# facebookresearch/robust_cvd

Hardware: AMD Instinct MI355X
Metric: GN/LM iterations/sec (and ms/iter) on 300-frame 384x224 video, 1/2/4/8 GPU (higher is better)
Workload: dtype f64

## Files before the change

robust_cvd_amd/csrc/cvd_host.h:

```cpp
#pragma once

#include <hip/hip_runtime.h>
#include <hip/hip_ext.h>
#include <rccl/rccl.h>
#include <rocblas/rocblas.h>
#include <rocsolver/rocsolver.h>

#include <algorithm>
#include <array>
#include <atomic>
#include <chrono>
#include <condition_variable>
#include <cmath>
#include <cstdarg>
#include <cstdint>
#include <cstdio>
#include <cstdlib>
#include <cstring>
#include <functional>
#include <limits>
#include <map>
#include <memory>
#include <mutex>
#include <set>
// ... 157 lines not shown
  DevBuf<float2> dDsrc, dDsrcOrd;
  int orderGx = -1, orderGy = -1;
  bool tableOrdered = false;
  DevBuf<unsigned char> dStatic, dInRange, dRegOwner;
  bool dense = false;
  DevBuf<float2> dFlow;
  DevBuf<unsigned char> dFMask;

  ncclComm_t comm = nullptr;
  int rank = 0, world = 1;
  std::shared_ptr<LocalGroup> localGroup;
  bool phantom = false;
  DevBuf<unsigned char> dCommStage;
  DevBuf<const unsigned char*> dCommPtrs;
  bool distForced = false;
  bool dist() const { return world > 1 || distForced; }
  int ownChunk() const { return (F + world - 1) / world; }
  int ownFirst() const { return std::min(F, rank * ownChunk()); }
  int ownCount() const { return std::min(F, (rank + 1) * ownChunk()) - ownFirst(); }
  int framesPadded() const { return dist() ? ownChunk() * world : F; }
  bool haveTriplets = false;
  std::vector<int> tripCenter;
  std::vector<long long> tripOff;
  long long tripC = 0;
  DevBuf<float> dTLoc, dTDsrc;
  DevBuf<float2> dTNdc;
  DevBuf<unsigned char> dTStatic;
  DevBuf<int> dTGroupOfC, dTCenterAll, dTCenter, dTSlot, dFtOff, dFtList;
  DevBuf<long long> dTOff;
  DevBuf<double> dCostTrip;
  std::vector<int> tripActive;
  bool tableWithTriplets = false;
  long long numValidTrip = 0;
  int qRows = 0;

  std::vector<int> itemFa, itemFb;
  std::vector<long long> itemRange;
  DevBuf<int> dItemFa, dItemFb, dItemSlot, dFiOff, dFiList, dFpOff, dFpList;
  DevBuf<AsmPart> dAsmParts;
  DevBuf<int2> dAsmUnits;
  DevBuf<double> dAsmScratch;
  DevBuf<unsigned int> dAsmCount;
  int nAsmParts = 0, nAsmSlots = 0;
  int numCU = 256;
  hipStream_t stream2 = nullptr;
  rocblas_handle rbMain = nullptr;
  DevBuf<double> dInvScratch;
  DevBuf<int> dInvInfo;
  hipEvent_t evCoarseIn = nullptr, evCoarseDone = nullptr;
  hipStream_t stream3 = nullptr;
  hipEvent_t evInvIn = nullptr, evInvDone = nullptr;
  DevBuf<FrameConst> dFc2;
  DevBuf<long long> dItemRange;
  std::vector<int> xFa, xFb;
  DevBuf<int> dXFa, dXFb, dXSlot, dXFiOff, dXPairEdge, dXDiagSlot;
  bool xDiagRows = false;
  int xRows = 0;
  DevBuf<long long> dXRange;
  DevBuf<double> dXBlocks;
  DevBuf<int> dDwPair, dDwRecOff, dXDir;
  DevBuf<double> dDwRecords, dDwGg;
  int nDwRecords = 0;
  bool denseAsList = false;
  bool denseListValid = false;
  std::vector<long long> denseListOff;
  DevBuf<int> dDlCounts;
  DevBuf<long long> dDlOffsets;
  DevBuf<unsigned int> dCounters;
  DevBuf<unsigned int> dTailBar;
  DevBuf<double> dOwnerScal;
  std::vector<unsigned char> tableRange;
  bool tableValid = false;
  bool tableIgnoresStatic = false;
  long long numValid = 0;

  std::vector<cvd_frame_pose> poses;
  cvd_xform_desc ddesc{}, sdesc{};
  std::vector<double> dparams, sparams;
  std::vector<std::array<double, 7>> poseParams;
  bool poseParamsValid = false;

  DevBuf<double> dX, dXc, dG, dLam, dMask, dScale, dDx, dR, dR1, dZ, dP0, dP1, dQ, dH, dQPart;
  DevBuf<float> dMinv;
  DevBuf<double> dFdot, dCostItem, dCostFrame, dScal, dHd, dFocal;
  DevBuf<double> dStatPart;
  DevBuf<unsigned char> dDynMask;
  DevBuf<double> dAdaptW;
  int dynW = 0, dynH = 0, adaptGx = 0, adaptGy = 0;
  bool haveDynMasks = false;
  std::shared_ptr<Frontend> frontend;

  struct CoarseHost {
    bool valid = false;
    int nEdges = 0, nBlocks = 0, nLevels = 0;
    std::vector<int> itemEdge;
    DevBuf<int> order, pos, levelPtr, levelCols, lvlBlkPtr, lvlBlks, blkCol, blkRow, colPtr, rowPtr, rowBlk, updPtr, updBlk,
        updA, updB, edgeBlk, edgeFa, edgeFb, wPtr, wRow, wtPtr, wtBlk, wtCol, wtFrame, wuPtr, wuL, wuW, itemEdgeDev, wSlot;
    DevBuf<double> edges, diag, Lb, Linv, Wb, rc, qc, y, c, dotPart, fdotY, wq, dropDiag;
    bool sparsified = false;
    bool temporalPose = false;
    int ptNn = 0, ptStepFrames = 0, ptN = 0, ptBlocks = 0;
    std::vector<int> edgeFaHost, edgeFbHost;
    DevBuf<int> ptA, ptB, ptPtr, ptList;
    DevBuf<double> ptMat, ptInv, ptR, ptT, ptDot, ptRec;
    DevBuf<TlStep> ptStepDev;
    std::vector<unsigned char> ptStepHost;
// ... 424 lines not shown
```

robust_cvd_amd/csrc/cvd_kernels.h:

```cpp
#pragma once

#include "cvd_device.h"

namespace cvd {

struct Table {
  const float4* ndc;
  const float2* dsrc;
  const int* pairA;
  const int* pairB;
  const long long* pairOff;
  const float2* flow;
  const unsigned char* fmask;
  const float* depth;
  int W, H;
  float sx, sy, invAspect;
};

__device__ __forceinline__ int densePixelOfLoc(const Table& T, float lx, float ly) {
  int px = static_cast<int>(__fmul_rn(lx, static_cast<float>(T.W)));
  int py = static_cast<int>(__fmul_rn(__fdiv_rn(ly, T.invAspect), static_cast<float>(T.H)));
  px = min(max(px, 0), T.W - 1);
  py = min(max(py, 0), T.H - 1);
  return py * T.W + px;
// ... 3 lines not shown
  if (!(isfinite(fx1) && isfinite(fy1))) return false;
  const int ix1 = static_cast<int>(__fadd_rn(fx1, 0.5f)), iy1 = static_cast<int>(__fadd_rn(fy1, 0.5f));
  if (ix1 < 0 || ix1 >= T.W || iy1 < 0 || iy1 >= T.H) return false;
  const float lx0 = __fmul_rn(static_cast<float>(ix), T.sx), ly0 = __fmul_rn(static_cast<float>(iy), T.sy);
  const float lx1 = __fmul_rn(fx1, T.sx), ly1 = __fmul_rn(fy1, T.sy);
  loc = make_float4(lx0, ly0, lx1, ly1);
  n.x = __fadd_rn(-1.f, __fmul_rn(2.f, lx0));
  n.y = __fsub_rn(1.f, __fdiv_rn(__fmul_rn(2.f, ly0), T.invAspect));
  n.z = __fadd_rn(-1.f, __fmul_rn(2.f, lx1));
  n.w = __fsub_rn(1.f, __fdiv_rn(__fmul_rn(2.f, ly1), T.invAspect));
  ai = densePixelOfLoc(T, lx0, ly0);
  bi = densePixelOfLoc(T, lx1, ly1);
  return true;
}
__device__ __forceinline__ bool denseConstraintRequest(const Table& T, int pix, int fa, int fb, float2 f, float4& n, float2& d) {
  const int iy = pix / T.W, ix = pix - iy * T.W;
  float4 loc;
  int ai, bi;
  d = make_float2(0.f, 0.f);
  if (!densePixelGeometry(T, ix, iy, f, loc, n, ai, bi)) return false;
  const size_t fs = static_cast<size_t>(T.W) * T.H;
  d.x = T.depth[fa * fs + ai];
  d.y = T.depth[fb * fs + bi];
  return true;
}
__device__ __forceinline__ bool denseDepthsValid(float2 d) { return isfinite(d.x) && d.x > 0.f && isfinite(d.y) && d.y > 0.f; }
__device__ __forceinline__ bool denseConstraintFromFlow(const Table& T, long long c, long long pixBase, int fa, int fb, float2 f,
                                                        float4& n, float2& d) {
  return denseConstraintRequest(T, static_cast<int>(c - pixBase), fa, fb, f, n, d) && denseDepthsValid(d);
}

template <bool DENSE>
__device__ __forceinline__ bool loadConstraint(const Table& T, long long c, long long pixBase, int fa, int fb, float4& n,
                                               float2& d) {
  if constexpr (!DENSE) {
    d = T.dsrc[c];
    n = T.ndc[c];
    return d.x > 0.f;
  } else {
    if (!T.fmask[c]) return false;
    return denseConstraintFromFlow(T, c, pixBase, fa, fb, T.flow[c], n, d);
  }
}

template <bool DENSE>
struct RecordStream {
  float4 ndNext;
  float2 dNext;
  __device__ __forceinline__ void prime(const Table& T, long long base, int i, int n) {
    ndNext = make_float4(0.f, 0.f, 0.f, 0.f);
    dNext = make_float2(0.f, 0.f);
    if (i < n) { dNext = (T.dsrc + base)[i]; ndNext = (T.ndc + base)[i]; }
  }
  __device__ __forceinline__ bool take(const Table& T, long long base, int i, int step, int n, long long, int, int, float4& nd,
                                       float2& d) {
    nd = ndNext;
    d = dNext;
    if (i + step < n) { dNext = (T.dsrc + base)[i + step]; ndNext = (T.ndc + base)[i + step]; }
    return d.x > 0.f;
  }
};
template <>
struct RecordStream<true> {
  float2 fNext;
  unsigned int mNext;
  __device__ __forceinline__ void prime(const Table& T, long long base, int i, int n) {
    fNext = make_float2(0.f, 0.f);
    mNext = 0u;
    if (i < n) { mNext = (T.fmask + base)[i]; fNext = (T.flow + base)[i]; }
  }
  __device__ __forceinline__ bool take(const Table& T, long long base, int i, int step, int n, long long pixBase, int fa, int fb,
                                       float4& nd, float2& d) {
    const unsigned int m = mNext;
    const float2 f = fNext;
    if (i + step < n) { mNext = (T.fmask + base)[i + step]; fNext = (T.flow + base)[i + step]; }
    if (!m) return false;
    return denseConstraintFromFlow(T, base + i, pixBase, fa, fb, f, nd, d);
  }
};

struct DenseStreamAhead {
  float2 fNext;
  unsigned int mNext;
  float4 ndCur;
  float2 dCur;
  bool candCur;
  __device__ __forceinline__ bool request(const Table& T, int pix, int fa, int fb, float2 f, float4& n, float2& d) const {
    return denseConstraintRequest(T, pix, fa, fb, f, n, d);
  }
  __device__ __forceinline__ void prime(const Table& T, long long base, int i, int step, int n, long long pixBase, int fa, int fb) {
    unsigned int m0 = 0u;
    float2 f0 = make_float2(0.f, 0.f);
    fNext = make_float2(0.f, 0.f);
    mNext = 0u;
    if (i < n) { m0 = (T.fmask + base)[i]; f0 = (T.flow + base)[i]; }
    if (i + step < n) { mNext = (T.fmask + base)[i + step]; fNext = (T.flow + base)[i + step]; }
    ndCur = make_float4(0.f, 0.f, 0.f, 0.f);
    candCur = m0 != 0u && request(T, static_cast<int>(base - pixBase) + i, fa, fb, f0, ndCur, dCur);
  }
  __device__ __forceinline__ bool take(const Table& T, long long base, int i, int step, int n, long long pixBase, int fa, int fb,
                                       float4& nd, float2& d) {
    nd = ndCur;
    d = dCur;
    const bool cand = candCur;
    const unsigned int m1 = mNext;
    const float2 f1 = fNext;
    mNext = 0u;
    if (i + 2 * step < n) { mNext = (T.fmask + base)[i + 2 * step]; fNext = (T.flow + base)[i + 2 * step]; }
    candCur = m1 != 0u && request(T, static_cast<int>(base - pixBase) + i + step, fa, fb, f1, ndCur, dCur);
    return cand && denseDepthsValid(d);
  }
};

struct Items {
  const int* fa;
  const int* fb;
  const long long* range;
  const int* slot;
  int count;
};

constexpr int kDenseFramesPerGroup = 2;
constexpr int kAsmUnit = 128;
constexpr int kAsmUnitDense = 1024;
constexpr int kDenseRun = 16;

#ifndef CVD_DETERMINISTIC
#define CVD_DETERMINISTIC 0
#endif
constexpr int kAtomicWalkers256 = CVD_DETERMINISTIC ? 64 : 256;
constexpr int kAsmThreads = CVD_DETERMINISTIC ? 64 : 512;
struct AsmPart {
  int frame;
  int u0, u1;
  int part;
  int nParts;
  int slot0;
};
struct AsmWork {
  const AsmPart* parts;
  const int2* units;
  double* scratch;
  unsigned int* counters;
};

__host__ __device__ inline int dwRecordDoubles(int G) { return 256 + 40 * G + 8; }
struct DenseRecords {
  const double* records;
  const int* recOff;
  const int* fpOff;
  const int* fpList;
};

enum : int { S_RZ = 0, S_RZOLD = 1, S_BETA = 2, S_PQ = 3, S_ALPHA = 4, S_RR = 5, S_RZ0 = 6, S_COST = 7,
             S_DG = 8, S_DR = 9, S_DLD = 10, S_DD = 11, S_XX = 12, S_NVALID = 13, S_GMAX = 14,
             S_DONE = 15, S_TARGET = 16, S_ITERS = 17,
             S_RZPART = 18,
             S_NACTIVE = 19,
             S_COUNT = 20 };

__device__ __forceinline__ double blockSumArray(const double* __restrict__ a, int n, double* red) {
  double acc = 0.0;
  for (int i = threadIdx.x; i < n; i += blockDim.x) acc += a[i];
  acc = waveSum(acc);
  __syncthreads();
  if ((threadIdx.x & 63) == 0) red[threadIdx.x >> 6] = acc;
  __syncthreads();
  double t = 0.0;
  for (int w = 0; w < (blockDim.x >> 6); ++w) t += red[w];
  __syncthreads();
  return t;
}
// ... 410 lines not shown
      dr2dDb = ((zIsMax ? 0.0 : dmx) + (zIsMin ? 0.0 : dmn)) * L.wd;
    } else {
      r2 = log(mn / mx) * L.wd;
      const double dmn = 1.0 / mn, dmx = -1.0 / mx;
      dr2dA = ((zIsMax ? dmx : 0.0) + (zIsMin ? dmn : 0.0)) * L.wd;
      dr2dDb = ((zIsMax ? 0.0 : dmx) + (zIsMin ? 0.0 : dmn)) * L.wd;
    }
  }
}

template <int SPEC>
__device__ __forceinline__ double fastRobustRho1(const Layout& L, double sq) {
  if constexpr (SPEC == 1) return rcpFast(1.0 + sq * L.cauchyC);
  else if constexpr (SPEC == 2) {
    const bool outer = sq > L.cauchyB;
    const double irt = rsqrtFast(outer ? sq : 1.0);
    return outer ? fmax(2.2250738585072014e-308, L.robustA * irt) : 1.0;
  }
  else return robustRho1(L, sq);
}
template <int SPEC>
__device__ __forceinline__ double fastRobustRho0(const Layout& L, double sq) {
  static_assert(SPEC == 1 || SPEC == 2, "the runtime choice goes through robustRho");
  if constexpr (SPEC == 1) {
    return L.cauchyB * log(1.0 + sq * L.cauchyC);
  } else {
    const bool outer = sq > L.cauchyB;
    const double irt = rsqrtFast(outer ? sq : 1.0);
    return outer ? (2.0 * L.robustA * (sq * irt) - L.cauchyB) : sq;
  }
}

__device__ __forceinline__ void fastRows(const Layout& L, double iz, double u, double vv, double ifxb, double ifyb, double& m00,
                                         double& m11, double& m02, double& m12) {
  const double wiz = L.ws * iz;
  m00 = wiz * ifxb;
  m11 = wiz * ifyb;
  m02 = wiz * u;
  m12 = wiz * vv;
}

#ifdef CVD_MV_PROFILE
__device__ unsigned long long g_mvProf[4096 * 8];
#define MV_STAMP(slot) do { if ((threadIdx.x & 63) == 0) g_mvProf[(blockIdx.x & 4095) * 8 + (slot)] = wall_clock64(); } while (0)
#else
#define MV_STAMP(slot) do {} while (0)
#endif
constexpr int kRedVals = 15;
constexpr int kRedStride = 4 * 33 + 1;

#ifndef CVD_MV_WAVES
#define CVD_MV_WAVES 4
#endif
#ifndef CVD_MV_SLOAD
#define CVD_MV_SLOAD 1
#endif
#ifndef CVD_MV_EARLY
#define CVD_MV_EARLY 1
#endif
template <int KD, int NT, int SPEC = 0, bool DENSE = false>
inline __global__ __launch_bounds__(NT) __attribute__((amdgpu_waves_per_eu(SPEC ? ((KD <= 4 && !DENSE) ? CVD_MV_WAVES : 3) : 2))) void k_matvec_pairs_fast(Layout L, Table T, Items it, const double* __restrict__ x,
                                                           const FrameConst* __restrict__ fc,
                                                           const double* __restrict__ mask,
                                                           const double* __restrict__ z, const double* __restrict__ pOld,
                                                           const double* __restrict__ scal, int useBeta,
                                                           double* __restrict__ qPart, CoarseView V) {
  const double sDone = scal[S_DONE];
  extern __shared__ __attribute__((aligned(16))) double sm[];
  constexpr int NV = KD == 1 ? kRedVals : 11;
  const int B = L.B;
  if (threadIdx.x == 0) MV_STAMP(0);
  double* xa = sm;
  double* xb = xa + B;
  double* pa = xb + B;
  double* pb = pa + B;
  double* qa = pb + B;
  double* qb = qa + B;
  FrameConst* fcs = reinterpret_cast<FrameConst*>(qb + B);
  double* red = reinterpret_cast<double*>(fcs + 2);
  double* W = red + 32;
  constexpr int kPriv = DENSE ? 8 : 1;
  constexpr bool kUsePriv = kPriv > 1;
  double* qpriv = W + static_cast<size_t>(kRedVals) * kRedStride;
  double* cl = W;
  const int item = blockIdx.x;
  const int tid = threadIdx.x;
  const int fa = it.fa[item], fb = it.fb[item];
  const double beta = useBeta ? scal[S_BETA] : 0.0;
#if CVD_MV_SLOAD
  const FrameConst* __restrict__ fcF[2] = {fc + fa, fc + fb};
#else
  const FrameConst* fcF[2] = {fcs, fcs + 1};
  {
    constexpr int FCW = sizeof(FrameConst) / 8;
    if (tid >= NT - 2 * FCW) {
      const int t = tid - (NT - 2 * FCW);
      const int which = t / FCW, k = t % FCW;
      reinterpret_cast<double*>(fcs + which)[k] = reinterpret_cast<const double*>(fc + (which ? fb : fa))[k];
    }
  }
#endif
  const long long cb0 = it.range[item * 4], ce0 = it.range[item * 4 + 1];
  constexpr bool kEarlyPrime = KD <= 4 && CVD_MV_EARLY;
  RecordStream<DENSE> rs;
  if constexpr (kEarlyPrime) rs.prime(T, cb0, (tid >> 6) * 64 + (tid & 63), static_cast<int>(ce0 - cb0));
  if (V.Wb != nullptr) {
    if (tid < 64) coarseFrameCorrection(V, fa, tid, cl);
    if (NT == 64) coarseFrameCorrection(V, fb, tid, cl + kCB);
    else if (tid >= 64 && tid < 128) coarseFrameCorrection(V, fb, tid - 64, cl + kCB);
  } else if (tid < 2 * kCB) {
    cl[tid] = (V.cF != nullptr) ? V.cF[(tid < kCB ? fa : fb) * kCB + (tid & (kCB - 1))] : 0.0;
  }
  constexpr int EPT = 256 / NT;
  double vza[EPT], vzb[EPT], vpa[EPT], vpb[EPT], vma[EPT], vmb[EPT];
  const bool tlOn = V.tl != nullptr;
  double* tls = cl + 2 * kCB;
  TlTaps tt[EPT];
  if (tlOn) {
    for (int i = tid; i < 2 * V.tlS; i += NT) {
      const int which = i >= V.tlS ? 1 : 0;
      tls[i] = V.tl[static_cast<size_t>(which ? fb : fa) * V.tlS + (i - which * V.tlS)];
    }
#pragma unroll
    for (int e = 0; e < EPT; ++e) tlLoadTaps(V, tid + e * NT, L.nD, tt[e]);
  }
#pragma unroll
  for (int e = 0; e < EPT; ++e) {
    const int i = tid + e * NT;
    vza[e] = vzb[e] = vpa[e] = vpb[e] = vma[e] = vmb[e] = 0.0;
    if (i < B) {
      const size_t ia = static_cast<size_t>(fa) * B + i, ib = static_cast<size_t>(fb) * B + i;
      xa[i] = x[ia];
      xb[i] = x[ib];
      vza[e] = z[ia];
      vzb[e] = z[ib];
      if (useBeta) { vpa[e] = pOld[ia]; vpb[e] = pOld[ib]; }
      vma[e] = mask[ia];
      vmb[e] = mask[ib];
      qa[i] = 0.0;
      qb[i] = 0.0;
    }
  }
  if constexpr (kUsePriv)
    for (int i = tid; i < kPriv * 2 * B; i += NT) qpriv[i] = 0.0;
  __syncthreads();
  if (sDone != 0.0) return;
#pragma unroll
  for (int e = 0; e < EPT; ++e) {
    const int i = tid + e * NT;
    if (i < B) {
      double ca = coarseAtLds(cl, L, i), cb2 = coarseAtLds(cl + kCB, L, i);
      if (tlOn) {
        ca += tlAt(tls, tt[e]);
        cb2 += tlAt(tls + V.tlS, tt[e]);
      }
      pa[i] = (vza[e] + ca + (useBeta ? beta * vpa[e] : 0.0)) * vma[e];
      pb[i] = (vzb[e] + cb2 + (useBeta ? beta * vpb[e] : 0.0)) * vmb[e];
    }
  }
  if (L.intrOpt == kIntrShared) {
    __syncthreads();
    if (tid == 0) {
      const double p06 = (z[6] + (useBeta ? beta * pOld[6] : 0.0)) * mask[6];
      pa[6] = p06;
      pb[6] = p06;
    }
  }
  __syncthreads();
  if (threadIdx.x == 0) MV_STAMP(1);

  const int N = SPEC ? 1 : L.N;
  const int lossType = SPEC ? static_cast<int>(kLossDisparity) : L.lossType;
  const double A = L.aspect;
  double aT[3] = {0, 0, 0}, aT0[3] = {0, 0, 0};
  double Cx[3] = {0, 0, 0};
  double aFa = 0.0, aFb = 0.0;
  double gDa[2] = {0.0, 0.0}, gDb[2] = {0.0, 0.0};
  const long long units0 = (it.range[item * 4 + 1] - it.range[item * 4] + 63) >> 6;
  for (int dir = 0; dir < 2; ++dir) {
  const long long cb = it.range[item * 4 + dir * 2], ce = it.range[item * 4 + dir * 2 + 1];
  const FrameConst& Fa = *fcF[dir];
  const FrameConst& Fb = *fcF[dir ^ 1];
  if (dir) {
    double* t;
    t = xa; xa = xb; xb = t;
    t = pa; pa = pb; pb = t;
    t = qa; qa = qb; qb = t;
#pragma unroll
    for (int i = 0; i < 3; ++i) { aT0[i] = aT[i]; aT[i] = 0.0; Cx[i] = -Cx[i]; }
    { const double o = aFa; aFa = aFb; aFb = o; }
#pragma unroll
    for (int n = 0; n < 2; ++n) { const double o = gDa[n]; gDa[n] = gDb[n]; gDb[n] = o; }
  }
  const int firstUnit = dir == 0 ? (tid >> 6) : static_cast<int>(((tid >> 6) - units0) & (NT / 64 - 1));
  const int nDir = static_cast<int>(ce - cb);
  const int iFirst = firstUnit * 64 + (tid & 63);
  if (dir || !kEarlyPrime) rs.prime(T, cb, iFirst, nDir);
  double RaU[9], RbU[9], dTU[3];
#pragma unroll
  for (int i = 0; i < 9; ++i) { RaU[i] = uniformValue(Fa.R[i]); RbU[i] = uniformValue(Fb.R[i]); }
#pragma unroll
  for (int i = 0; i < 3; ++i) dTU[i] = uniformValue(Fa.t[i] - Fb.t[i]);
  double eaU[3], ebU[3], dptU[3];
  {
    const double pwa[3] = {uniformValue(pa[3]), uniformValue(pa[4]), uniformValue(pa[5])};
    const double pwb[3] = {uniformValue(pb[3]), uniformValue(pb[4]), uniformValue(pb[5])};
#pragma unroll
    for (int k = 0; k < 3; ++k) {
      eaU[k] = uniformValue(pwa[0] * Fa.Jl[k] + pwa[1] * Fa.Jl[3 + k] + pwa[2] * Fa.Jl[6 + k]);
      ebU[k] = uniformValue(pwb[0] * Fb.Jl[k] + pwb[1] * Fb.Jl[3 + k] + pwb[2] * Fb.Jl[6 + k]);
      dptU[k] = uniformValue(pa[k] - pb[k]);
    }
  }
  const double fya = uniformValue(Fa.fy), fxa = fya * A;
  const double fyb = uniformValue(Fb.fy);
  const double ifyb = uniformValue(1.0 / fyb), ifxb = uniformValue(1.0 / (fyb * A));
  const double pfaU = uniformValue(pa[6] / fya);
  const double pfrU = uniformValue(L.ws * pb[6] * ifyb);

  const int fsrc = dir ? fb : fa, ftgt = dir ? fa : fb;
  const long long pixBase = DENSE ? (cb / (static_cast<long long>(T.W) * T.H)) * (static_cast<long long>(T.W) * T.H) : 0;
  for (int ci = iFirst; ci < nDir; ci += NT) {
    float4 nd;
    float2 d;
    if (!rs.take(T, cb, ci, NT, nDir, pixBase, fsrc, ftgt, nd, d)) continue;
    const double da = static_cast<double>(d.x), db = static_cast<double>(d.y);
    FastTaps<KD> ta, tb;
    fastGather<KD>(L, nd.x, nd.y, ta);
    fastGather<KD>(L, nd.z, nd.w, tb);
    double Da, Db, sDa, sDb;
    if (N == 0) {
      Da = da; Db = db; sDa = 0.0; sDb = 0.0;
    } else {
// ... 52 lines not shown

    const double yq0 = m00 * t0, yq1 = m11 * t1, yq2 = m02 * t0 + m12 * t1 - dr2dA * t2;
    aFb -= L.ws * (u * t0 + vv * t1);
    const double yX[3] = {RbU[0] * yq0 + RbU[1] * yq1 + RbU[2] * yq2, RbU[3] * yq0 + RbU[4] * yq1 + RbU[5] * yq2,
                          RbU[6] * yq0 + RbU[7] * yq1 + RbU[8] * yq2};
#pragma unroll
    for (int i = 0; i < 3; ++i) aT[i] += yX[i];
    Cx[0] += v[1] * yX[2] - v[2] * yX[1];
    Cx[1] += v[2] * yX[0] - v[0] * yX[2];
    Cx[2] += v[0] * yX[1] - v[1] * yX[0];
    aFa += Da * (Rcf[0] * yX[0] + Rcf[1] * yX[1] + Rcf[2] * yX[2]);
    if (N > 0) {
      const double ga = Rca[0] * yX[0] + Rca[1] * yX[1] + Rca[2] * yX[2];
      const double gb = dr2dDb * t2;
      float dxLate = d.x, dyLate = d.y;
      asm volatile("" : "+v"(dxLate), "+v"(dyLate));
      const double da = static_cast<double>(dxLate), db = static_cast<double>(dyLate);
      if constexpr (KD == 1) {
        gDa[0] += ga * da; gDa[1] += ga;
        gDb[0] += gb * db; gDb[1] += gb;
      } else {
      const int pkey = (DENSE ? tid : (tid ^ (tid >> 5))) & (kPriv - 1);
      double* qaw = kUsePriv ? qpriv + (static_cast<size_t>(pkey) * 2 + dir) * B : qa;
      double* qbw = kUsePriv ? qpriv + (static_cast<size_t>(pkey) * 2 + (dir ^ 1)) * B : qb;
      const double gad = ga * da, gbd = gb * db;
#pragma unroll
      for (int k = 0; k < KD; ++k) {
        if (ta.ok(k)) {
          const int ia = ta.I(k);
          const double wa = ta.Wt(k);
          if (N == 2) {
            atomicAdd(&qaw[7 + ia * 2], gad * wa);
            atomicAdd(&qaw[7 + ia * 2 + 1], ga * wa);
          } else {
            atomicAdd(&qaw[7 + ia], gad * wa);
          }
        }
        if (tb.ok(k)) {
          const int ib = tb.I(k);
          const double wb = tb.Wt(k);
          if (N == 2) {
            atomicAdd(&qbw[7 + ib * 2], gbd * wb);
            atomicAdd(&qbw[7 + ib * 2 + 1], gb * wb);
          } else {
            atomicAdd(&qbw[7 + ib], gbd * wb);
          }
        }
      }
      }
    }
  }
  }
  MV_STAMP(4 + ((threadIdx.x >> 6) & 3));
  const FrameConst& Fa = *fcF[1];
  const FrameConst& Fb = *fcF[0];
  {
    double vals[NV];
#pragma unroll
    for (int i = 0; i < 3; ++i) { vals[i] = aT[i]; vals[3 + i] = aT0[i]; vals[6 + i] = Cx[i]; }
    vals[9] = aFa;
    vals[10] = aFb;
    if constexpr (KD == 1) { vals[11] = gDa[0]; vals[12] = gDa[1]; vals[13] = gDb[0]; vals[14] = gDb[1]; }
    const int half = tid >> 1;
    const int colw = (half >> 5) * 33 + (half & 31);
#pragma unroll
    for (int i = 0; i < NV; ++i) {
      const double v = vals[i] + dppMove<0xB1>(vals[i]);
      if ((tid & 1) == 0) W[i * kRedStride + colw] = v;
    }
  }
  __syncthreads();
  constexpr int SEG = NT / 64;
  if (tid < NV * SEG) {
    const double* row = W + (tid / SEG) * kRedStride + (tid % SEG) * 33;
    double s0 = 0.0, s1 = 0.0, s2 = 0.0, s3 = 0.0;
#pragma unroll
    for (int k = 0; k < 32; k += 4) {
      s0 += row[k];
      s1 += row[k + 1];
      s2 += row[k + 2];
      s3 += row[k + 3];
    }
    double sacc = (s0 + s1) + (s2 + s3);
    if (SEG >= 2) sacc += dppMove<0xB1>(sacc);
    if (SEG == 4) sacc += dppMove<0x4E>(sacc);
    if (tid % SEG == 0) red[tid / SEG] = sacc;
  }
  __syncthreads();
  if (tid < 3) {
    const double d = red[tid] - red[3 + tid];
    qa[tid] += d;
    qb[tid] -= d;
  } else if (tid < 9) {
    const bool tgt = tid >= 6;
    const int i = tgt ? tid - 6 : tid - 3;
    const double dT[3] = {Fa.t[0] - Fb.t[0], Fa.t[1] - Fb.t[1], Fa.t[2] - Fb.t[2]};
    const double* y = red + (tgt ? 3 : 0);
    const double m[3] = {red[6] - (dT[1] * y[2] - dT[2] * y[1]), red[7] - (dT[2] * y[0] - dT[0] * y[2]),
                         red[8] - (dT[0] * y[1] - dT[1] * y[0])};
    const double* a = (tgt ? Fb.Jl : Fa.Jl) + 3 * i;
    const double sdot = a[0] * m[0] + a[1] * m[1] + a[2] * m[2];
    if (tgt) qb[3 + i] -= sdot;
    else qa[3 + i] += sdot;
  } else if (tid == 9) {
    qa[6] += red[9] / Fa.fy;
  } else if (tid == 10) {
    qb[6] += red[10] / Fb.fy;
  } else if (KD == 1 && tid < 15) {
    const int n = (tid - 11) & 1;
    if (n < N) {
      if (tid < 13) qa[7 + n] += red[11 + n];
      else qb[7 + n] += red[13 + n];
    }
  }
  __syncthreads();
  if (threadIdx.x == 0) MV_STAMP(2);
  { double* t = qa; qa = qb; qb = t; }
  if constexpr (kUsePriv) {
    for (int i = tid; i < B; i += NT) {
      double sa = 0.0, sb = 0.0;
#pragma unroll
      for (int k = 0; k < kPriv; ++k) {
        sa += qpriv[(static_cast<size_t>(k) * 2 + 0) * B + i];
        sb += qpriv[(static_cast<size_t>(k) * 2 + 1) * B + i];
      }
      qa[i] += sa;
      qb[i] += sb;
    }
    __syncthreads();
  }
  double* outA = qPart + static_cast<size_t>(it.slot[item * 2]) * B;
  double* outB = qPart + static_cast<size_t>(it.slot[item * 2 + 1]) * B;
  for (int i = tid; i < B; i += NT) {
    outA[i] = qa[i];
    outB[i] = qb[i];
  }
  if (threadIdx.x == 0) MV_STAMP(3);
}

}
```

robust_cvd_amd/csrc/cvd_setup.hip:

```cpp
#include "cvd_host.h"
#include "cvd_table.h"
#include "cvd_triplets.h"
#include "cvd_dense_walk.h"
#include <rocprim/device/device_segmented_radix_sort.hpp>

namespace cvd {

void launchFrameConsts(const Layout& L, const double* x, FrameConst* fc, hipStream_t s) {
  hipLaunchKernelGGL(k_frame_consts, dim3((L.F + 63) / 64), dim3(64), 0, s, L, x, fc);
}

static void quatToMatrix(const double q[4] , double R[3][3]) {
  for (int c = 0; c < 3; ++c) {
    double v[3] = {0, 0, 0};
    v[c] = 1.0;
    const double uv[3] = {2.0 * (q[1] * v[2] - q[2] * v[1]), 2.0 * (q[2] * v[0] - q[0] * v[2]),
                          2.0 * (q[0] * v[1] - q[1] * v[0])};
    R[0][c] = v[0] + q[3] * uv[0] + (q[1] * uv[2] - q[2] * uv[1]);
    R[1][c] = v[1] + q[3] * uv[1] + (q[2] * uv[0] - q[0] * uv[2]);
    R[2][c] = v[2] + q[3] * uv[2] + (q[0] * uv[1] - q[1] * uv[0]);
  }
}
static void matrixToAngleAxis(const double R[3][3], double aa[3]) {
  double q0, q1, q2, q3;
// ... 902 lines not shown
    const bool overBudget = coarseEliminationUpdates(h->F, edgeList) > updateBudget;
    {
      const int stepP = std::max(2, h->opt.coarse_temporal_step);
      const bool fits = ((h->F - 1 + stepP - 1) / stepP + 1) * kCB <= kDenseCoarseMaxUnknowns;
      const bool fusedScope = !h->dist() && h->opt.pcg_fused_tail != 0 && !h->forceGeneric && h->Bsz() <= 256 &&
                              h->opt.coarse_temporal_min_frames > 0 && h->F >= h->opt.coarse_temporal_min_frames &&
                              h->F + 2 * kTlMaxS <= 2 * h->numCU;
      h->coarse.temporalPose = fits && (h->opt.coarse_level == 3 || (overBudget && h->opt.coarse_over_budget == 0) ||
                                        (h->opt.coarse_over_budget == 0 && fusedScope));
    }
    if (h->coarse.temporalPose) {
      h->coarse.denseMode = true;
    } else if (overBudget && h->F * kCB <= denseMaxUnknowns) {
      h->coarse.denseMode = true;
    } else if (overBudget) {
      std::vector<int> newId(edgeList.size(), -1);
      std::vector<std::pair<int, int>> kept;
      for (size_t e = 0; e < edgeList.size(); ++e)
        if (coarseKeepsPair(edgeList[e].first, edgeList[e].second)) {
          newId[e] = static_cast<int>(kept.size());
          kept.push_back(edgeList[e]);
        }
      for (auto& ie : itemEdge) ie = newId[ie];
      h->coarse.sparsified = kept.size() != edgeList.size();
      edgeList.swap(kept);
    }
    buildCoarsePlan(h, edgeList, itemEdge);
    if (h->coarse.temporalPose) poseTemporalPlan(h);
    if (h->dense) {
      std::map<std::pair<int, int>, int> edgeOfPair;
      for (size_t i = 0; i < h->itemFa.size(); ++i) edgeOfPair[{h->itemFa[i], h->itemFb[i]}] = itemEdge[i];
      std::vector<int> pairEdge(std::max<size_t>(1, h->xFa.size()), -1);
      for (size_t k = 0; k < h->xFa.size(); ++k) {
        auto it = edgeOfPair.find({h->xFa[k], h->xFb[k]});
        if (it != edgeOfPair.end()) pairEdge[k] = it->second;
      }
      h->dXPairEdge.upload(pairEdge.data(), pairEdge.size(), s);
    }
  }
  std::vector<int> fiOff(h->F + 1, 0), fiList, fpOff(h->F + 1, 0), fpList;
  for (int f = 0; f < h->F; ++f) {
    fiOff[f + 1] = fiOff[f] + static_cast<int>(frameItems[f].size());
    fiList.insert(fiList.end(), frameItems[f].begin(), frameItems[f].end());
    fpOff[f + 1] = fpOff[f] + static_cast<int>(framePairs[f].size());
    fpList.insert(fpList.end(), framePairs[f].begin(), framePairs[f].end());
  }
  h->dItemFa.upload(h->itemFa.data(), h->itemFa.size(), s);
  h->dItemFb.upload(h->itemFb.data(), h->itemFb.size(), s);
  h->dItemRange.upload(h->itemRange.data(), h->itemRange.size(), s);
  std::vector<int> itemSlot(fiList.size(), 0);
  for (size_t e = 0; e < fiList.size(); ++e) itemSlot[fiList[e]] = static_cast<int>(e);
  h->qRows = static_cast<int>(fiList.size());
  h->dItemSlot.upload(itemSlot.data(), itemSlot.size(), s);
  if (withTriplets) {
    const size_t nG = h->tripActive.size();
    std::vector<long long> tOff(2 * std::max<size_t>(nG, 1), 0);
    std::vector<int> tCen(std::max<size_t>(nG, 1), 0), tSlot(3 * std::max<size_t>(nG, 1), 0);
    const int pairCodes = static_cast<int>(h->itemFa.size()) * 2;
    for (size_t k = 0; k < nG; ++k) {
      const int g = h->tripActive[k];
      tOff[2 * k] = h->tripOff[g];
      tOff[2 * k + 1] = h->tripOff[g + 1];
      tCen[k] = h->tripCenter[g];
      for (int role = 0; role < 3; ++role) tSlot[3 * k + role] = itemSlot[pairCodes + static_cast<int>(k) * 3 + role];
    }
    std::vector<int> ftOff(h->F + 1, 0), ftList;
    for (int f = 0; f < h->F; ++f) {
      ftOff[f + 1] = ftOff[f] + static_cast<int>(frameTrips[f].size());
      ftList.insert(ftList.end(), frameTrips[f].begin(), frameTrips[f].end());
    }
    h->dTOff.upload(tOff.data(), tOff.size(), s);
    h->dTCenter.upload(tCen.data(), tCen.size(), s);
    h->dTSlot.upload(tSlot.data(), tSlot.size(), s);
    h->dFtOff.upload(ftOff.data(), ftOff.size(), s);
    h->dFtList.upload(ftList.data(), ftList.size(), s);
    h->dCostTrip.ensure(std::max<size_t>(nG, 1));
  }
  {
    std::vector<int2> units;
    std::vector<int> fuOff(h->F + 1, 0);
    for (int f = 0; f < h->F; ++f) {
      for (const int code : framePairs[f]) {
        const long long n = h->pairOff[(code >> 1) + 1] - h->pairOff[code >> 1];
        for (long long o = 0; o < n; o += (h->dense ? kAsmUnitDense : kAsmUnit)) units.push_back(make_int2(code, static_cast<int>(o)));
      }
      fuOff[f + 1] = static_cast<int>(units.size());
    }
    int activeFrames = 0;
    for (int f = 0; f < h->F; ++f) activeFrames += inRange[f] ? 1 : 0;
    constexpr double partsPerCU = 1.0;
    const long long denom = std::max<long long>(1, std::max<long long>(activeFrames, static_cast<long long>(partsPerCU * h->numCU)));
    const int capU = static_cast<int>(std::max<long long>(kAsmThreads / 64, (static_cast<long long>(units.size()) + denom - 1) / denom));
    std::vector<AsmPart> parts;
    int slots = 0;
    for (int f = 0; f < h->F; ++f) {
      const int nu = fuOff[f + 1] - fuOff[f];
      const int np = std::max(1, (nu + capU - 1) / capU);
      const int per = (nu + np - 1) / np;
      for (int q = 0; q < np; ++q) {
        AsmPart a;
        a.frame = f;
        a.u0 = fuOff[f] + std::min(nu, q * per);
        a.u1 = fuOff[f] + std::min(nu, (q + 1) * per);
        a.part = q;
        a.nParts = np;
        a.slot0 = np > 1 ? slots : 0;
// ... 189 lines not shown
```

robust_cvd_amd/csrc/cvd_solve.hip:

```cpp
#include <optional>

#include "cvd_host.h"
#include "cvd_lm.h"
#include "cvd_pcg.h"
#include "cvd_coarse.h"

namespace cvd {

void launchTlRowsInit(cvd_handle* h, const TlStep* tsp, int NT, int groups, int F, unsigned int* counter, int closeScalars, double tol2,
                      hipStream_t s) {
  const size_t lds = static_cast<size_t>(tlRowsLds(NT)) * 8;
  allowLds(k_tl_rows_init, lds);
  hipLaunchKernelGGL(k_tl_rows_init, dim3(groups), dim3(768), lds, s, tsp, F, h->dScal.p, counter, closeScalars, tol2, h->hPcg);
  HIP_CHECK(hipGetLastError());
}

namespace {
struct TailStalled {};
}
static int runPcgAttempt(Ctx& c, const double* x, const std::function<void()>& tail);
int runPcg(Ctx& c, const double* x, const std::function<void()>& tail) {
  const size_t firstTimerSlot = c.h->evUsed;
  try {
    return runPcgAttempt(c, x, tail);
// ... 198 lines not shown
bool wantsTriplets(const cvd_opt_params& p, ProblemKind kind) {
  return kind == PK_POSE_STEP && (p.smooth_static_weight > 0.0 || p.smooth_dynamic_weight > 0.0);
}
void bindTriplets(Ctx& c, const cvd_opt_params& p, ProblemKind kind) {
  cvd_handle* h = c.h;
  c.trip = wantsTriplets(p, kind) && c.L.includeStatic;
  if (!c.trip) return;
  c.TT = TripletTable{h->dTNdc.p, h->dTDsrc.p, h->dTStatic.p, h->dTOff.p, h->dTCenter.p, h->dTSlot.p,
                      static_cast<int>(h->tripActive.size()),
                      static_cast<int>(p.smooth_loss_type),
                      std::sqrt(std::max(0.0, p.smooth_static_weight)), std::sqrt(std::max(0.0, p.smooth_dynamic_weight))};
}

namespace {

struct SetupPhases {
  bool on;
  double t = nowSeconds();
  void operator()(const char* what) {
    if (!on) return;
    const double now = nowSeconds();
    fprintf(stderr, "[setup] %-14s %8.1f us\n", what, (now - t) * 1e6);
    t = now;
  }
};

struct BindMode {
  bool checkBlock;
  bool staticGuards;
  bool levels;
};
struct BoundProblem {
  Ctx c;
  std::optional<DenseListScope> denseList;
};

void bindProblem(BoundProblem& b, cvd_handle* h, const cvd_opt_params& p, double depthDeformReg, ProblemKind kind,
                 const std::vector<int>& range, const BindMode& mode, SetupPhases& phase) {
  Ctx& c = b.c;
  c.h = h;
  c.L = makeLayout(h, p, depthDeformReg, kind);
  if (mode.checkBlock) checkFrameBlock(static_cast<size_t>(c.L.B), "solve");
  tapCounts(c.L, c.KD, c.KS);
  phase("layout");
  const bool guarded = !mode.staticGuards || c.L.includeStatic;
  b.denseList.emplace(h, h->dense && guarded && !denseFastScope(h, c.L, c.KS, wantsTriplets(p, kind)));
  compileTable(h, range, wantsTriplets(p, kind), kind == PK_NORMALIZE && c.L.includeStatic);
  orderTable(h, c.L, c.KD);
  phase("table");
  refreshMedians(h);
  phase("medians");
  c.T = makeTable(h);
  c.nItems = static_cast<int>(h->itemFa.size());
  c.it = Items{h->dItemFa.p, h->dItemFb.p, h->dItemRange.p, h->dItemSlot.p, c.nItems};
  c.n = static_cast<size_t>(c.L.F) * c.L.B;
  c.boundDepth0 = (kind == PK_NORMALIZE && c.L.N > 0) ? 1 : 0;
  bindTriplets(c, p, kind);
  if (guarded) checkDenseScope(h, c.L, c.KS, c.trip);
  c.cross = crossScope(h, c);
  h->coarseOn = mode.levels && h->opt.coarse_level != 0 && h->coarse.valid && c.L.includeStatic && h->coarse.nEdges > 0 &&
                !h->forceGeneric && kind == PK_POSE_STEP;
  ensureBuffers(c);
  phase("buffers");
  if (mode.levels) {
    h->coarse.ptInvPending = false;
    h->temporal.on = temporalScope(c);
    if (h->temporal.on) h->temporal.on = temporalPrepare(c);
    phase("level 3 tables");
    if (h->coarseOn && h->coarse.temporalPose) poseTemporalPrepare(c);
    phase("level 2 tables");
  }
  buildMask(h, c.L, p, kind, range);
  phase("mask");
  uploadState(h, c.L, h->dX);
  phase("upload");
}

long long countResidualBlocks(const Ctx& c, const std::vector<int>& range) {
  const cvd_handle* h = c.h;
  const long long nr = static_cast<long long>(range.size());
  long long blocks = c.trip ? h->numValidTrip : 0;
  if (c.L.scaleRegSqrt > 0.0) blocks += nr * c.L.sregX * c.L.sregY;
  if (c.L.focalRegSqrt > 0.0) blocks += nr;
  if (c.L.depthDeformW > 0.0 && c.L.depthType == CVD_DEPTH_GRID) blocks += nr;
  if (c.L.spatialDeformW > 0.0 && c.L.nS > 0) blocks += nr;
  if (c.L.positionRegSqrt > 0.0)
    for (int k = c.L.firstFrame; k < c.L.lastFrame - 1; ++k)
      blocks += (h->tableRange[k] && h->tableRange[k + 1] && h->tableRange[k + 2]) ? 1 : 0;
  return blocks;
}

struct PendingGuard {
  cvd_handle* h;
  const LevelSchedule& schedule;
  bool inverseAside = false;
  ~PendingGuard() {
    if (schedule.pending) (void)hipStreamWaitEvent(h->stream, h->evCoarseDone, 0);
    if (inverseAside) (void)hipStreamWaitEvent(h->stream, h->evInvDone, 0);
    if (h->temporal.sidePending) {
      (void)hipStreamWaitEvent(h->stream, h->temporal.evDone, 0);
      h->temporal.sidePending = false;
    }
  }
};

void rebuildTemporalLevel(Ctx& c) {
  cvd_handle* h = c.h;
// ... 296 lines not shown
```

Before: 327.1.

## Pack per-item metadata into one cache-line record and hoist matvec prologue loads

Per-item frame indices, output slots and constraint ranges now live in one 64-byte aligned record, so the matvec kernel reads them from one cache line instead of several scattered arrays. The kernel prologue now issues every global load up front into registers before writing shared memory: x/z/pOld/mask rows, coarse and temporal coefficients, tap data and the needed FrameConst fields (t, fy, Jl). Clamped addresses keep those loads branch-free. The aim is to overlap load latency at kernel start. In exchange it adds register pressure, unconditional loads of unused data, and an extra setup upload of the record array.

Result: faster. 333.1, median of 6 (+1.8%).

```diff
diff --git a/robust_cvd_amd/csrc/cvd_host.h b/robust_cvd_amd/csrc/cvd_host.h
--- a/robust_cvd_amd/csrc/cvd_host.h
+++ b/robust_cvd_amd/csrc/cvd_host.h
@@ -233,6 +233,7 @@
   hipEvent_t evInvIn = nullptr, evInvDone = nullptr;
   DevBuf<FrameConst> dFc2;
   DevBuf<long long> dItemRange;
+  DevBuf<ItemRecord> dItemRec;
   std::vector<int> xFa, xFb;
   DevBuf<int> dXFa, dXFb, dXSlot, dXFiOff, dXPairEdge, dXDiagSlot;
   bool xDiagRows = false;
diff --git a/robust_cvd_amd/csrc/cvd_kernels.h b/robust_cvd_amd/csrc/cvd_kernels.h
--- a/robust_cvd_amd/csrc/cvd_kernels.h
+++ b/robust_cvd_amd/csrc/cvd_kernels.h
@@ -79,6 +79,12 @@
     dNext = make_float2(0.f, 0.f);
     if (i < n) { dNext = (T.dsrc + base)[i]; ndNext = (T.ndc + base)[i]; }
   }
+  __device__ __forceinline__ void primeClamped(const Table& T, long long base, int i, int n) {
+    const long long c = i < n ? base + i : 0;
+    dNext = T.dsrc[c];
+    ndNext = T.ndc[c];
+    if (i >= n) { dNext = make_float2(0.f, 0.f); ndNext = make_float4(0.f, 0.f, 0.f, 0.f); }
+  }
   __device__ __forceinline__ bool take(const Table& T, long long base, int i, int step, int n, long long, int, int, float4& nd,
                                        float2& d) {
     nd = ndNext;
@@ -96,6 +102,7 @@
     mNext = 0u;
     if (i < n) { mNext = (T.fmask + base)[i]; fNext = (T.flow + base)[i]; }
   }
+  __device__ __forceinline__ void primeClamped(const Table& T, long long base, int i, int n) { prime(T, base, i, n); }
   __device__ __forceinline__ bool take(const Table& T, long long base, int i, int step, int n, long long pixBase, int fa, int fb,
                                        float4& nd, float2& d) {
     const unsigned int m = mNext;
@@ -139,12 +146,21 @@
   }
 };
 
+struct alignas(64) ItemRecord {
+  int fa, fb;
+  int slotA, slotB;
+  long long b0, e0;
+  long long b1, e1;
+  long long pad[2];
+};
+static_assert(sizeof(ItemRecord) == 64, "one record per 64-byte line");
 struct Items {
   const int* fa;
   const int* fb;
   const long long* range;
   const int* slot;
   int count;
+  const ItemRecord* rec;
 };
 
 constexpr int kDenseFramesPerGroup = 2;
@@ -661,9 +677,6 @@
 #ifndef CVD_MV_WAVES
 #define CVD_MV_WAVES 4
 #endif
-#ifndef CVD_MV_SLOAD
-#define CVD_MV_SLOAD 1
-#endif
 #ifndef CVD_MV_EARLY
 #define CVD_MV_EARLY 1
 #endif
@@ -685,8 +698,8 @@
   double* pb = pa + B;
   double* qa = pb + B;
   double* qb = qa + B;
-  FrameConst* fcs = reinterpret_cast<FrameConst*>(qb + B);
-  double* red = reinterpret_cast<double*>(fcs + 2);
+  double* fix = qb + B;
+  double* red = fix + 2 * sizeof(FrameConst) / 8;
   double* W = red + 32;
   constexpr int kPriv = DENSE ? 8 : 1;
   constexpr bool kUsePriv = kPriv > 1;
@@ -694,58 +707,87 @@
   double* cl = W;
   const int item = blockIdx.x;
   const int tid = threadIdx.x;
-  const int fa = it.fa[item], fb = it.fb[item];
+  const ItemRecord* __restrict__ recp = it.rec + item;
+  const int fa = recp->fa, fb = recp->fb;
+  const int slotA = recp->slotA, slotB = recp->slotB;
+  const long long cbD[2] = {recp->b0, recp->b1}, ceD[2] = {recp->e0, recp->e1};
   const double beta = useBeta ? scal[S_BETA] : 0.0;
-#if CVD_MV_SLOAD
   const FrameConst* __restrict__ fcF[2] = {fc + fa, fc + fb};
-#else
-  const FrameConst* fcF[2] = {fcs, fcs + 1};
-  {
-    constexpr int FCW = sizeof(FrameConst) / 8;
-    if (tid >= NT - 2 * FCW) {
-      const int t = tid - (NT - 2 * FCW);
-      const int which = t / FCW, k = t % FCW;
-      reinterpret_cast<double*>(fcs + which)[k] = reinterpret_cast<const double*>(fc + (which ? fb : fa))[k];
-    }
-  }
-#endif
-  const long long cb0 = it.range[item * 4], ce0 = it.range[item * 4 + 1];
   constexpr bool kEarlyPrime = KD <= 4 && CVD_MV_EARLY;
   RecordStream<DENSE> rs;
-  if constexpr (kEarlyPrime) rs.prime(T, cb0, (tid >> 6) * 64 + (tid & 63), static_cast<int>(ce0 - cb0));
-  if (V.Wb != nullptr) {
+  if constexpr (kEarlyPrime) rs.primeClamped(T, cbD[0], tid, static_cast<int>(ceD[0] - cbD[0]));
+  constexpr int EPT = 256 / NT;
+  constexpr int TLE = (2 * kTlMaxS + NT - 1) / NT;
+  const bool fusedCoarse = V.Wb != nullptr;
+  const bool tlOn = V.tl != nullptr;
+  const size_t rowA = static_cast<size_t>(fa) * B, rowB = static_cast<size_t>(fb) * B;
+  double vcf;
+  {
+    const int k = tid & (2 * kCB - 1);
+    vcf = *(V.cF != nullptr ? V.cF + static_cast<size_t>(k < kCB ? fa : fb) * kCB + (k & (kCB - 1)) : x);
+  }
+  double* tls = cl + 2 * kCB;
+  double vtl[TLE];
+#pragma unroll
+  for (int e = 0; e < TLE; ++e) {
+    const int i = tid + e * NT;
+    const int ic = (tlOn && i < 2 * V.tlS) ? i : 0;
+    const int which = ic >= V.tlS ? 1 : 0;
+    vtl[e] = *(tlOn ? V.tl + static_cast<size_t>(which ? fb : fa) * V.tlS + (ic - which * V.tlS) : x);
+  }
+  TlTaps tt[EPT];
+#pragma unroll
+  for (int e = 0; e < EPT; ++e) {
+    const int i = tid + e * NT;
+    const bool in = i >= 7 && i < 7 + L.nD;
+    const int v = in ? i - 7 : 0;
+    tt[e].w = *(tlOn ? V.tlW + v : reinterpret_cast<const float4*>(x));
+    tt[e].idx = *(tlOn ? V.tlIdx + v : reinterpret_cast<const unsigned int*>(x));
+    if (!in) tt[e].w = make_float4(0.f, 0.f, 0.f, 0.f);
+  }
+  constexpr int kFix = 13;
+  static_assert(offsetof(FrameConst, fy) == offsetof(FrameConst, t) + 24 && offsetof(FrameConst, Jl) == offsetof(FrameConst, t) + 32,
+                "t, fy, Jl are consecutive");
+  const int fixK = NT - 1 - tid;
+  double vfix;
+  {
+    const int k = fixK < 2 * kFix ? fixK : 0;
+    vfix = (reinterpret_cast<const double*>(fc + (k >= kFix ? fb : fa)) + offsetof(FrameConst, t) / 8)[k >= kFix ? k - kFix : k];
+  }
+  double vxa[EPT], vxb[EPT], vza[EPT], vzb[EPT], vpa[EPT], vpb[EPT], vma[EPT], vmb[EPT];
+  const double* __restrict__ pOldOrZ = useBeta ? pOld : z;
+#pragma unroll
+  for (int e = 0; e < EPT; ++e) {
+    const int i = tid + e * NT;
+    const size_t ia = rowA + (i < B ? i : 0), ib = rowB + (i < B ? i : 0);
+    vxa[e] = x[ia];
+    vxb[e] = x[ib];
+    vza[e] = z[ia];
+    vzb[e] = z[ib];
+    vpa[e] = pOldOrZ[ia];
+    vpb[e] = pOldOrZ[ib];
+    vma[e] = mask[ia];
+    vmb[e] = mask[ib];
+  }
+  const double z6 = z[6], po6 = pOldOrZ[6], m6 = mask[6];
+  if (fusedCoarse) {
     if (tid < 64) coarseFrameCorrection(V, fa, tid, cl);
     if (NT == 64) coarseFrameCorrection(V, fb, tid, cl + kCB);
     else if (tid >= 64 && tid < 128) coarseFrameCorrection(V, fb, tid - 64, cl + kCB);
-  } else if (tid < 2 * kCB) {
-    cl[tid] = (V.cF != nullptr) ? V.cF[(tid < kCB ? fa : fb) * kCB + (tid & (kCB - 1))] : 0.0;
-  }
-  constexpr int EPT = 256 / NT;
-  double vza[EPT], vzb[EPT], vpa[EPT], vpb[EPT], vma[EPT], vmb[EPT];
-  const bool tlOn = V.tl != nullptr;
-  double* tls = cl + 2 * kCB;
-  TlTaps tt[EPT];
-  if (tlOn) {
-    for (int i = tid; i < 2 * V.tlS; i += NT) {
-      const int which = i >= V.tlS ? 1 : 0;
-      tls[i] = V.tl[static_cast<size_t>(which ? fb : fa) * V.tlS + (i - which * V.tlS)];
-    }
-#pragma unroll
-    for (int e = 0; e < EPT; ++e) tlLoadTaps(V, tid + e * NT, L.nD, tt[e]);
-  }
+  }
+  if (!fusedCoarse && tid < 2 * kCB) cl[tid] = (V.cF != nullptr) ? vcf : 0.0;
+#pragma unroll
+  for (int e = 0; e < TLE; ++e) {
+    const int i = tid + e * NT;
+    if (tlOn && i < 2 * V.tlS) tls[i] = vtl[e];
+  }
+  if (fixK < 2 * kFix) fix[fixK] = vfix;
 #pragma unroll
   for (int e = 0; e < EPT; ++e) {
     const int i = tid + e * NT;
-    vza[e] = vzb[e] = vpa[e] = vpb[e] = vma[e] = vmb[e] = 0.0;
     if (i < B) {
-      const size_t ia = static_cast<size_t>(fa) * B + i, ib = static_cast<size_t>(fb) * B + i;
-      xa[i] = x[ia];
-      xb[i] = x[ib];
-      vza[e] = z[ia];
-      vzb[e] = z[ib];
-      if (useBeta) { vpa[e] = pOld[ia]; vpb[e] = pOld[ib]; }
-      vma[e] = mask[ia];
-      vmb[e] = mask[ib];
+      xa[i] = vxa[e];
+      xb[i] = vxb[e];
       qa[i] = 0.0;
       qb[i] = 0.0;
     }
@@ -770,7 +812,7 @@
   if (L.intrOpt == kIntrShared) {
     __syncthreads();
     if (tid == 0) {
-      const double p06 = (z[6] + (useBeta ? beta * pOld[6] : 0.0)) * mask[6];
+      const double p06 = (z6 + (useBeta ? beta * po6 : 0.0)) * m6;
       pa[6] = p06;
       pb[6] = p06;
     }
@@ -785,9 +827,9 @@
   double Cx[3] = {0, 0, 0};
   double aFa = 0.0, aFb = 0.0;
   double gDa[2] = {0.0, 0.0}, gDb[2] = {0.0, 0.0};
-  const long long units0 = (it.range[item * 4 + 1] - it.range[item * 4] + 63) >> 6;
+  const long long units0 = (ceD[0] - cbD[0] + 63) >> 6;
   for (int dir = 0; dir < 2; ++dir) {
-  const long long cb = it.range[item * 4 + dir * 2], ce = it.range[item * 4 + dir * 2 + 1];
+  const long long cb = cbD[dir], ce = ceD[dir];
   const FrameConst& Fa = *fcF[dir];
   const FrameConst& Fb = *fcF[dir ^ 1];
   if (dir) {
@@ -946,8 +988,8 @@
   }
   }
   MV_STAMP(4 + ((threadIdx.x >> 6) & 3));
-  const FrameConst& Fa = *fcF[1];
-  const FrameConst& Fb = *fcF[0];
+  const double* fixFa = fix + kFix;
+  const double* fixFb = fix;
   {
     double vals[NV];
 #pragma unroll
@@ -988,18 +1030,18 @@
   } else if (tid < 9) {
     const bool tgt = tid >= 6;
     const int i = tgt ? tid - 6 : tid - 3;
-    const double dT[3] = {Fa.t[0] - Fb.t[0], Fa.t[1] - Fb.t[1], Fa.t[2] - Fb.t[2]};
+    const double dT[3] = {fixFa[0] - fixFb[0], fixFa[1] - fixFb[1], fixFa[2] - fixFb[2]};
     const double* y = red + (tgt ? 3 : 0);
     const double m[3] = {red[6] - (dT[1] * y[2] - dT[2] * y[1]), red[7] - (dT[2] * y[0] - dT[0] * y[2]),
                          red[8] - (dT[0] * y[1] - dT[1] * y[0])};
-    const double* a = (tgt ? Fb.Jl : Fa.Jl) + 3 * i;
+    const double* a = (tgt ? fixFb : fixFa) + 4 + 3 * i;
     const double sdot = a[0] * m[0] + a[1] * m[1] + a[2] * m[2];
     if (tgt) qb[3 + i] -= sdot;
     else qa[3 + i] += sdot;
   } else if (tid == 9) {
-    qa[6] += red[9] / Fa.fy;
+    qa[6] += red[9] / fixFa[3];
   } else if (tid == 10) {
-    qb[6] += red[10] / Fb.fy;
+    qb[6] += red[10] / fixFb[3];
   } else if (KD == 1 && tid < 15) {
     const int n = (tid - 11) & 1;
     if (n < N) {
@@ -1023,8 +1065,8 @@
     }
     __syncthreads();
   }
-  double* outA = qPart + static_cast<size_t>(it.slot[item * 2]) * B;
-  double* outB = qPart + static_cast<size_t>(it.slot[item * 2 + 1]) * B;
+  double* outA = qPart + static_cast<size_t>(slotA) * B;
+  double* outB = qPart + static_cast<size_t>(slotB) * B;
   for (int i = tid; i < B; i += NT) {
     outA[i] = qa[i];
     outB[i] = qb[i];
diff --git a/robust_cvd_amd/csrc/cvd_setup.hip b/robust_cvd_amd/csrc/cvd_setup.hip
--- a/robust_cvd_amd/csrc/cvd_setup.hip
+++ b/robust_cvd_amd/csrc/cvd_setup.hip
@@ -978,6 +978,13 @@
   for (size_t e = 0; e < fiList.size(); ++e) itemSlot[fiList[e]] = static_cast<int>(e);
   h->qRows = static_cast<int>(fiList.size());
   h->dItemSlot.upload(itemSlot.data(), itemSlot.size(), s);
+  {
+    std::vector<ItemRecord> rec(std::max<size_t>(1, h->itemFa.size()), ItemRecord{});
+    for (size_t i = 0; i < h->itemFa.size(); ++i)
+      rec[i] = ItemRecord{h->itemFa[i], h->itemFb[i], itemSlot[2 * i], itemSlot[2 * i + 1], h->itemRange[4 * i], h->itemRange[4 * i + 1],
+                          h->itemRange[4 * i + 2], h->itemRange[4 * i + 3], {0, 0}};
+    h->dItemRec.upload(rec.data(), rec.size(), s);
+  }
   if (withTriplets) {
     const size_t nG = h->tripActive.size();
     std::vector<long long> tOff(2 * std::max<size_t>(nG, 1), 0);
diff --git a/robust_cvd_amd/csrc/cvd_solve.hip b/robust_cvd_amd/csrc/cvd_solve.hip
--- a/robust_cvd_amd/csrc/cvd_solve.hip
+++ b/robust_cvd_amd/csrc/cvd_solve.hip
@@ -274,7 +274,7 @@
   phase("medians");
   c.T = makeTable(h);
   c.nItems = static_cast<int>(h->itemFa.size());
-  c.it = Items{h->dItemFa.p, h->dItemFb.p, h->dItemRange.p, h->dItemSlot.p, c.nItems};
+  c.it = Items{h->dItemFa.p, h->dItemFb.p, h->dItemRange.p, h->dItemSlot.p, c.nItems, h->dItemRec.p};
   c.n = static_cast<size_t>(c.L.F) * c.L.B;
   c.boundDepth0 = (kind == PK_NORMALIZE && c.L.N > 0) ? 1 : 0;
   bindTriplets(c, p, kind);
```
